# Zilong-Li/BaseVarC

Measured on AMD Instinct MI355X. Metric: sites/sec at N=1e6 samples; achieved HBM GB/s vs roofline, higher is better.
Workload: dtype f64

## Files before the change

### basevarc_amd/csrc/bvc_internal.h

```cpp
#pragma once
#include <hip/hip_runtime.h>
#include <stdint.h>

#include <vector>

#include "../../include/bvc.h"

namespace bvc {

struct LaunchState {
    int n_cu = 256;
    int em_waves_per_cu = 0;
    int em_wpb = 4;
    int hist_split = 0;
    int host_chunk_kib = 1 << 19;
    int em_streams = 0;
    int group_pipe = 1;
    int group_log2c = -1;
    int group_big_lds = 1;
    int group_h16 = 0;
    int em_engine = 0;
    int em_tiny_regions = 0;
    int csr_scatter_max = 64;
    int em_prune = 1;
    int stats_log2c = 2;
    int dbg_levels = 0;
    mutable uint32_t em_epoch = 0;
    struct RaisedLds { const void *kernel; size_t bytes; };
    mutable std::vector<RaisedLds> lds_raised;
};

inline size_t round256(size_t n) { return (n + 255) / 256 * 256; }

struct Layout {
    uintptr_t base = 0;
    size_t at = 0;
    template <class T> T *take(size_t count, size_t pad = 0)
    {
        T *p = reinterpret_cast<T *>(base + at);
        at += round256(count * sizeof(T) + pad);
        return p;
    }
};

hipError_t raise_lds(const LaunchState &st, const void *kernel, size_t bytes);

struct QualLut {
    double a[128];
    double e[128];
    double e_empty;
    double log_e[128];
    double log_a[128];
};

hipError_t launch_hist_dense(LaunchState &st, hipStream_t stream, int64_t n_sites, int64_t n_samples, int64_t row_stride,
                             const int8_t *bases, const int8_t *quals, const uint8_t *group_of_sample,
                             int n_groups, uint32_t *counts, int split, int64_t *group_scratch = nullptr,
                             uint8_t *hist_of_sample = nullptr);
constexpr int kGroupScratchWords = BVC_MAX_GROUPS + 4;
inline size_t group_redo_offset(int64_t n_samples) { return ((size_t)n_samples + 255) & ~(size_t)255; }
inline size_t group_labels_bytes(int64_t n_samples, int64_t n_sites) { return group_redo_offset(n_samples) + (size_t)n_sites + 256; }
int choose_hist_split(const LaunchState &st, int64_t n_sites, int64_t n_samples);

hipError_t launch_hist_packed(LaunchState &st, hipStream_t stream, int64_t n_sites, int64_t n_samples, int64_t row_stride,
                              const uint8_t *packed, uint32_t *counts, int split);
hipError_t launch_hist_packed_groups(LaunchState &st, hipStream_t stream, int64_t n_sites, int64_t n_samples,
                                     int64_t row_stride, const uint8_t *packed, const uint8_t *group_of_sample, int n_groups,
                                     uint32_t *counts, int64_t *group_scratch, uint8_t *hist_of_sample);
hipError_t launch_pack_dense(hipStream_t stream, int64_t n_sites, int64_t n_samples, int64_t stride_in, const int8_t *bases,
                             const int8_t *quals, int64_t stride_out, uint8_t *packed, unsigned long long *bad);

hipError_t launch_stream_read(hipStream_t stream, const void *src, int64_t bytes, uint32_t *sink);

hipError_t launch_hist_csr(LaunchState &st, hipStream_t stream, int64_t n_sites, const int64_t *offsets,
                           const int8_t *bases, const int8_t *quals, uint32_t *counts);

inline bool uses_item_engine(const LaunchState &st, double min_af) { return st.em_engine != 1 && min_af > 0.0; }
hipError_t launch_lrt(const LaunchState &st, hipStream_t stream, int64_t n_sites, const uint32_t *counts,
                      int64_t hist_stride, const int8_t *ref_base, double min_af, const QualLut *lut,
                      const int8_t *comb, const uint8_t *n_comb, bvc_site_result *results, bool shared = false,
                      int shared_waves_per_cu = 0,
                      void *scratch = nullptr);

size_t em_items_scratch_bytes(int64_t n_sites);
hipError_t launch_lrt_items(const LaunchState &st, hipStream_t stream, int64_t n_sites, int n_groups,
                            const uint32_t *counts, int64_t hist_stride, const int8_t *ref_base, double min_af,
                            const QualLut *lut, const int8_t *comb, const uint8_t *n_comb, bvc_site_result *results,
                            void *scratch, const uint8_t **taken_out, bool shared = false);

hipError_t launch_lrt_groups(const LaunchState &st, hipStream_t stream, int64_t n_sites, int n_groups,
                             const uint32_t *grp_counts, const int8_t *ref_base, double min_af, const QualLut *lut,
                             const bvc_site_result *overall, bvc_group_result *grp_results, bool shared = false,
                             int shared_waves_per_cu = 0, void *scratch = nullptr);
size_t em_group_scratch_bytes(int64_t n_sites, int n_groups);
constexpr int kGroupSharedWavesPerCu = 8;

hipError_t launch_sum_groups(hipStream_t stream, int64_t n_sites, int n_hist, const uint32_t *grp_counts,
                             uint32_t *counts);

hipError_t launch_synth_dense(hipStream_t stream, uint64_t seed, int64_t site0, int64_t n_sites,
                              int64_t n_samples, int64_t row_stride, uint32_t cov_thr16,
                              int8_t *bases, int8_t *quals, int8_t *ref_base);

struct PileupTile {
    const uint8_t *text = nullptr;
    bool bin = false;
    const uint32_t *line_start = nullptr;
    const int32_t *sample0 = nullptr, *n_in_batch = nullptr;
    int32_t n_batches = 0, n_pos = 0;
    int32_t line_stride = 0;
    const int32_t *n_pos_dev = nullptr;
    int64_t n_lines_cap = 0;
    uint32_t *line_words = nullptr;
    uint32_t *status = nullptr;
    int64_t *entry_off = nullptr, *obs_off = nullptr, *totals = nullptr;
    bvc_pileup_entry *entries = nullptr;
    int32_t *samples = nullptr;
    int8_t *obs_base = nullptr, *obs_qual = nullptr;
    const uint8_t *group_of_sample = nullptr;
    int64_t n_samples = 0;
    int32_t n_groups = 0;
    uint8_t *obs_label = nullptr;
    int32_t *tally = nullptr;
    bvc_pileup_indel *indels = nullptr;
    uint32_t indel_cap = 0;
};
struct bvc_pileup_region { uint32_t start, len, left_src, left_len; };
hipError_t launch_region_carry(hipStream_t stream, const uint8_t *old_text, uint8_t *text, const bvc_pileup_region *regions, int32_t n_batches);
hipError_t launch_region_index(hipStream_t stream, const PileupTile &P, const bvc_pileup_region *regions, const uint32_t *seg_base,
                               int64_t n_segments, uint32_t *seg_nl, int32_t *lines, int32_t max_pos);
hipError_t launch_region_ends(hipStream_t stream, const PileupTile &P, uint32_t *ends);
hipError_t launch_indel_text(hipStream_t stream, const PileupTile &P, uint8_t *dst, uint32_t dst_cap, uint32_t *used);
hipError_t launch_called_scan(hipStream_t stream, const PileupTile &P, const bvc_site_result *results, int64_t *called_off);
hipError_t launch_called_gather(hipStream_t stream, const PileupTile &P, const int64_t *called_off, bvc_pileup_entry *out_entries,
                                int32_t *out_samples);
hipError_t launch_pileup_count(hipStream_t stream, const PileupTile &P);
hipError_t launch_pileup_write(hipStream_t stream, const PileupTile &P, uint32_t carry_in);
hipError_t launch_hist_csr_groups(LaunchState &st, hipStream_t stream, int64_t n_sites, const int64_t *offsets, const int8_t *bases,
                                  const int8_t *quals, const int32_t *sample_of_obs, const uint8_t *group_of_sample, int64_t n_samples,
                                  int n_groups, uint32_t *counts);
hipError_t launch_hist_csr_labels(LaunchState &st, hipStream_t stream, int64_t n_sites, const int64_t *offsets, const uint8_t *obs,
                                  const uint8_t *quals, const uint8_t *group_of_obs, int n_groups, uint32_t *counts);

hipError_t launch_counts_add(hipStream_t stream, int64_t n_words, uint32_t *dst, const uint32_t *src);
hipError_t launch_hist_csr_scatter(const LaunchState &st, hipStream_t stream, int64_t n_sites, const int64_t *offsets, const uint8_t *obs,
                                   const uint8_t *quals, const uint8_t *group_of_obs, int n_groups, int64_t max_len, uint32_t *counts);
hipError_t launch_hist_csr_add(LaunchState &st, hipStream_t stream, int64_t n_sites, const int64_t *offsets, const uint8_t *obs,
                               const uint8_t *quals, const uint8_t *group_of_obs, int n_groups, int64_t min_len, uint32_t *counts);

constexpr int kStatsMaxLog2c = 4;
constexpr int kSiteStatsTrip = 4096;
hipError_t launch_site_stats(LaunchState &st, hipStream_t stream, int64_t n_sites, const int64_t *offsets, const bvc_pileup_entry *entries,
                             const int8_t *ref_base, const bvc_site_result *results, bvc_site_stats *stats);

hipError_t launch_inflate(hipStream_t stream, const uint8_t *comp, const bvc_bgzf_block *blocks, int64_t n_blocks, uint8_t *out, uint32_t *status);

#ifdef BVC_CHECK_LDS
hipError_t debug_read_inflate(uint32_t *out8, bool reset);
hipError_t debug_read_pileup(uint32_t *out8, bool reset);
hipError_t debug_read_site_stats(uint32_t *out8, bool reset);
hipError_t debug_read_hist(uint32_t *out8, bool reset);
hipError_t debug_read_wave_engine(uint32_t *out8, bool reset);
hipError_t debug_read_items(uint32_t *out8, bool reset);
#endif

}
```

### basevarc_amd/csrc/em_items.hip

```cpp
#include <algorithm>

#include "bvc_device.h"
#include "bvc_internal.h"
#include "em_common.h"

namespace bvc {
namespace {



constexpr int kTiny = 8, kNarrow = 32, kWide = 48;
template <int CPB> constexpr int site_table_bytes() { return 4 * CPB * 5; }

constexpr int kEmptyQ = 128;

struct FitItem {
    int32_t site;
    uint8_t base[4];
    double f0[4];
    double e_excl;
    double inv_n;
    double ll_excl;
};
static_assert(sizeof(FitItem) == 64, "FitItem layout");
// ... 420 lines not shown
        const FitItem *fi = items + item;
        const int base = fi->base[unit];
        if (base != 0xFF && BVC_LDS_OK(13, fi->site, kRegionSites) && BVC_LDS_OK(14, base, 4)) {
            active = true;
            fb = fi->f0[unit];
            const uint8_t *tab = cls + fi->site * site_table_bytes<CPB>();
            const uint32_t *tab_n = reinterpret_cast<const uint32_t *>(tab) + base * CPB + sub;
            const uint8_t *tab_q = tab + 16 * CPB + base * CPB + sub;
#pragma unroll
            for (int k = 0; k < kSlots; ++k) {
                n[k] = (double)tab_n[k * G];
                e[k] = lut_e[tab_q[k * G]];
            }
        }
    }
    if (!active) {
#pragma unroll
        for (int k = 0; k < kSlots; ++k) { n[k] = 0.0; e[k] = 0.25; }
    }

    double fprev = fb, dprev = 0.0;
    int it = 0;
    bool done = !valid;
    while (true) {
        double ta = fabs(fb - fprev) * dprev;
        const double e_excl = fi_c->e_excl, fb_scale = fi_c->inv_n;
        const double g = fma(-4.0, fb, 1.0);
        double ysum0 = 0.0, ysum1 = 0.0, acc_e0 = 0.0, acc_e1 = 0.0;
#ifdef BVC_RCP_CHUNK
        constexpr int CH = kSlots > BVC_RCP_CHUNK ? BVC_RCP_CHUNK : kSlots;
#else
        constexpr int CH = kSlots;
#endif
#pragma unroll
        for (int c0 = 0; c0 < kSlots; c0 += CH) {
            constexpr int kLast = kSlots % CH == 0 ? CH : kSlots % CH;
            if (c0 + CH <= kSlots) {
                double m[CH], y[CH];
#pragma unroll
                for (int k = 0; k < CH; ++k) m[k] = fma(g, e[c0 + k], fb);
                rcp_all<CH>(m, y);
#pragma unroll
                for (int k = 0; k < CH; k += 2) {
                    const double r0 = n[c0 + k] * y[k], r1 = n[c0 + k + 1] * y[k + 1];
                    ysum0 += r0; ysum1 += r1;
                    acc_e0 = fma(r0, e[c0 + k], acc_e0); acc_e1 = fma(r1, e[c0 + k + 1], acc_e1);
                }
            } else {
                double m[kLast], y[kLast];
#pragma unroll
                for (int k = 0; k < kLast; ++k) m[k] = fma(g, e[c0 + k], fb);
                rcp_all<kLast>(m, y);
#pragma unroll
                for (int k = 0; k < kLast; k += 2) {
                    const double r0 = n[c0 + k] * y[k], r1 = n[c0 + k + 1] * y[k + 1];
                    ysum0 += r0; ysum1 += r1;
                    acc_e0 = fma(r0, e[c0 + k], acc_e0); acc_e1 = fma(r1, e[c0 + k + 1], acc_e1);
                }
            }
        }
        const double acc_e = acc_e0 + acc_e1;
        const double acc_d = fma(-4.0, acc_e, ysum0 + ysum1);
        double etot = acc_e;
        item_sum2<ROWS, LOG2G>(etot, ta);
        const double dunit = unit_sum<LOG2G>(acc_d);
        const double ex = (fb * fb_scale) * (dunit + (etot + e_excl));
        const uint32_t a_hi = (uint32_t)__double2hiint(ta);
        bool conv = it > 0 && a_hi < kSureBelowHi;
        const bool straddle = !done && it > 0 && a_hi >= kSureBelowHi && a_hi < kSureAboveHi;
        if (__ballot(straddle) != 0) {
            double dl = 0.0;
            const double df = fb - fprev, gp = fma(-4.0, fprev, 1.0);
#pragma unroll
            for (int k = 0; k < kSlots; ++k) {
                const double mo = fma(gp, e[k], fprev);
                const double u = df * fma(-4.0, e[k], 1.0) * rcp_cubic(mo);
                double p = fma(-0.25, u, 1.0 / 3.0);
                p = fma(p, u, -0.5);
                p = fma(p, u, 1.0);
                dl = fma(n[k], fabs(u * p), dl);
            }
            dl = item_sum<ROWS, LOG2G>(dl);
            conv = conv || (straddle && dl < kEmEpsilon);
        }
        const bool stop = !done && (conv || it == kEmIters);
        if (__ballot(stop) != 0) {
            if (stop && sub == 0) {
                FitOut *o = outs + item;
                o->ex[unit] = active ? ex : 0.0;
                o->fl[unit] = fb;
                if (ROWS == 2) o->ex[unit + 2] = 0.0;
                if (unit == 0) { o->passes = it + 1; o->pad = 0; }
            }
            done = done || stop;
            if (__ballot(!done) == 0) break;
        }
        fprev = fb;
        dprev = acc_d;
        fb = ex;
        ++it;
    }
    {
        const double fl = outs[valid ? item : item0].fl[unit];
        const double g = fma(-4.0, fl, 1.0);
        double ll = 0.0;
#pragma unroll
        for (int k = 0; k < kSlots; ++k) {
            ll = fma(n[k], log_pos(fma(g, e[k], fl)), ll);
            if ((k & 3) == 3) __builtin_amdgcn_sched_barrier(0);
        }
        ll = item_sum<ROWS, LOG2G>(ll);
        if (valid && unit == 0 && sub == 0) outs[item].ll = ll + items[item].ll_excl;
    }
}

constexpr int kLog2G4 = 1, kLog2G2 = 2;
template <int CPB> constexpr int log2g4() { return CPB == kTiny ? 0 : kLog2G4; }
template <int CPB> constexpr int log2g2() { return CPB == kTiny ? 1 : kLog2G2; }
constexpr double kPruneSlackAbs = 1.0, kPruneSlackRel = 1e-6;

template <class RegionT>
__device__ __forceinline__ void site_decide(RegionT &R, int ls, int lane, int64_t site, int n_groups, int prune,
                                            const int8_t *__restrict__ ref_base, bvc_site_result *__restrict__ results)
{
    ItemSite S = R.site[ls];
    if (S.state != 1) {
        int zero = 0;
        asm volatile("" : "+v"(zero));
        if (lane == 0) { R.want[ls][0] = zero; R.want[ls][1] = zero; R.site[ls].n_emit = 0; }
        return;
    }
    uint32_t sets = 0;
    int n_emit = 0, p_deepest = 0;
    bool finished = false;

    auto fit_loglik = [&](int idx, double (&ex)[4], int &passes) -> double {
        if (!BVC_LDS_OK(15, idx, kPlaces)) idx = 0;
        const FitOut &o = R.outs[idx];
#pragma unroll
        for (int u = 0; u < 4; ++u) ex[u] = o.ex[u];
        passes = o.passes;
        return o.ll;
    };
    auto by_base = [&](uint32_t pm, const double (&ex)[4], double (&bp)[4]) {
#pragma unroll
        for (int j = 0; j < 4; ++j) bp[j] = 0.0;
        int u = 0;
#pragma unroll
        for (int p = 0; p < 4; ++p)
            if ((pm >> p) & 1u) {
                const int b = (S.blist >> (4 * p)) & 3u;
                const double v = u == 0 ? ex[0] : (u == 1 ? ex[1] : (u == 2 ? ex[2] : ex[3]));
                bp[0] = b == 0 ? v : bp[0]; bp[1] = b == 1 ? v : bp[1];
                bp[2] = b == 2 ? v : bp[2]; bp[3] = b == 3 ? v : bp[3];
                ++u;
            }
    };

    int first_sub = 0;
    if (S.first) {
        double ex[4];
        int passes = 0;
        S.lr_alt = fit_loglik(S.item[0], ex, passes);
        by_base((1u << S.n) - 1u, ex, S.base_frq);
        S.passes += passes; S.fits += 1;
        first_sub = 1;
        S.k = (int8_t)(S.n - 1);
        S.first = 0;
    }
    const int n = S.n, k = S.k;
    bool again = false;
    if (k < 1) {
        finished = true;
    } else if (k >= 2) {
        const int c_last = n - 1 - S.p_deepest;
        int i_min = S.best_i;
        double best_chi = S.best_chi, best_lr = S.best_lr;
        double best_bp[4] = {S.best_bp[0], S.best_bp[1], S.best_bp[2], S.best_bp[3]};
        if (!S.round2) {
            const uint32_t masks = S.sets >> (4 * first_sub);
            const int cnt = S.n_emit - first_sub;
#pragma unroll
            for (int c = 0; c < 3; ++c) {
                if (c >= cnt) break;
                const uint32_t pm = (masks >> (4 * c)) & 0xFu;
                double ex[4];
                int passes = 0;
                const double ll = fit_loglik(first_sub ? S.item[c + 1] : S.item[c], ex, passes);
                S.passes += passes; S.fits += 1;
                const double chi_c = 2.0 * (S.lr_alt - ll);
                if (c == 0 || chi_c < best_chi) {
                    best_chi = chi_c; best_lr = ll; i_min = (S.later && c >= c_last) ? c + 1 : c;
                    by_base(pm, ex, best_bp);
                }
            }
            if (S.later) {
                double u_c = 0.0;
                uint32_t in_set = 0;
#pragma unroll
                for (int p = 0; p < 4; ++p)
                    if ((S.later >> p) & 1u) in_set |= 1u << ((S.blist >> (4 * p)) & 3u);
#pragma unroll
                for (int b = 0; b < 4; ++b) u_c += ((in_set >> b) & 1u) ? 0.0 : S.lle[b];
                const double bound = 2.0 * (S.lr_alt - u_c);
                const bool ruled_out = prune && bound > best_chi + (kPruneSlackAbs + kPruneSlackRel * fabs(u_c)) && bound < __builtin_huge_val();
                again = !ruled_out;
            }
        } else {
            double ex[4];
            int passes = 0;
            const double ll = fit_loglik(S.item[0], ex, passes);
            S.passes += passes; S.fits += 1;
            const double chi_c = 2.0 * (S.lr_alt - ll);
            if (chi_c < best_chi || (chi_c == best_chi && c_last < i_min)) {
                best_chi = chi_c; best_lr = ll; i_min = c_last;
                by_base(S.later, ex, best_bp);
            }
        }
        if (again) {
            S.best_chi = best_chi; S.best_lr = best_lr; S.best_i = (int8_t)i_min;
#pragma unroll
            for (int j = 0; j < 4; ++j) S.best_bp[j] = best_bp[j];
            S.round2 = 1;
            sets = S.later; n_emit = 1; p_deepest = S.p_deepest;
        } else {
            S.round2 = 0;
            S.lr_alt = best_lr;
            S.chi = best_chi;
            if (best_chi < kLrtThreshold) {
                int cnt_all = 0;
                const uint32_t pm = (subset_masks(n, k, cnt_all) >> (4 * i_min)) & 0xFu;
                uint32_t nl = 0;
                int nn = 0;
#pragma unroll
                for (int p = 0; p < 4; ++p)
                    if ((pm >> p) & 1u) { nl |= ((S.blist >> (4 * p)) & 3u) << (4 * nn); ++nn; }
                S.blist = nl;
                S.n = (int8_t)k;
#pragma unroll
                for (int j = 0; j < 4; ++j) S.base_frq[j] = best_bp[j];
                S.k = (int8_t)(k - 1);
                S.later = 0;
                if (k - 1 >= 2) {
                    uint32_t later = 0;
                    p_deepest = deepest_position(S.depth, nl, k);
                    sets = level_subsets(k, p_deepest, n_emit, later);
                    S.later = (uint8_t)later;
                }
            } else {
                finished = true;
            }
        }
    }
    if (!finished && !again && S.k == 1) {
        const int b0 = (int)(S.blist & 3u), b1 = (int)((S.blist >> 4) & 3u);
        const double ll0 = single_allele_loglik(S.lla, S.lle, b0), ll1 = single_allele_loglik(S.lla, S.lle, b1);
        const double chi0 = 2.0 * (S.lr_alt - ll0), chi1 = 2.0 * (S.lr_alt - ll1);
        const bool second = chi1 < chi0;
        const double best_chi = second ? chi1 : chi0;
        const int bb = second ? b1 : b0;
        S.passes += 4; S.fits += 2;
        S.lr_alt = second ? ll1 : ll0;
        S.chi = best_chi;
        if (best_chi < kLrtThreshold) {
            S.blist = (uint32_t)bb;
            S.n = 1;
            S.base_frq[0] = bb == 0 ? 1.0 : 0.0; S.base_frq[1] = bb == 1 ? 1.0 : 0.0;
            S.base_frq[2] = bb == 2 ? 1.0 : 0.0; S.base_frq[3] = bb == 3 ? 1.0 : 0.0;
        }
        S.k = 0;
        finished = true;
    }
    S.sets = sets; S.n_emit = (int8_t)n_emit; S.p_deepest = (int8_t)p_deepest;
    int want[kLists];
    count_wanted(sets, n_emit, want);
    if (lane == 0) {
        if (finished) {
            store_record(results + site, S, (int)ref_base[ref_index(site, n_groups)], S.n, S.blist);
            S.state = 2;
        }
        R.site[ls] = S;
        R.want[ls][0] = want[0]; R.want[ls][1] = want[1];
    }
}

struct RegionArgs {
    int64_t n_sites;
    int n_groups;
    const uint32_t *counts;
    int64_t hist_stride;
    const QualLut *lut;
    const int8_t *ref_base;
    double min_af;
    const int8_t *comb;
    const uint8_t *n_comb;
    uint8_t *taken;
    bvc_site_result *results;
    uint32_t *kind_epoch;
    uint32_t epoch;
    int dbg_levels;
    int tiny_regions;
    int prune;
    int64_t region0;
};

__device__ __forceinline__ void wave_sync()
{
    __builtin_amdgcn_fence(__ATOMIC_RELEASE, "workgroup");
    __builtin_amdgcn_wave_barrier();
    __builtin_amdgcn_fence(__ATOMIC_ACQUIRE, "workgroup");
}

__device__ __forceinline__ void load_counts(uint32_t (&c)[8], const uint32_t *__restrict__ counts, int64_t hist_stride, int64_t site,
                                            int n_groups, int lane)
{
    const uint32_t *hist = counts + hist_index(site, n_groups) * hist_stride + (lane >> 4) * 128 + (lane & 15);
#pragma unroll
    for (int lvl = 0; lvl < 8; ++lvl) c[lvl] = hist[16 * lvl];
}

template <int TEAM, class RegionT>
__device__ __forceinline__ void team_sync(RegionT &R, uint32_t &phase, int lane)
{
    if (TEAM == 1) { wave_sync(); return; }
    __builtin_amdgcn_fence(__ATOMIC_RELEASE, "workgroup");
    __builtin_amdgcn_wave_barrier();
    phase += TEAM;
    if (lane == 0) {
        __hip_atomic_fetch_add(&R.arrive, 1u, __ATOMIC_RELEASE, __HIP_MEMORY_SCOPE_WORKGROUP);
        while (__hip_atomic_load(&R.arrive, __ATOMIC_ACQUIRE, __HIP_MEMORY_SCOPE_WORKGROUP) - phase > 0x7FFFFFFFu) __builtin_amdgcn_s_sleep(1);
    }
    __builtin_amdgcn_wave_barrier();
    __builtin_amdgcn_fence(__ATOMIC_ACQUIRE, "workgroup");
}

template <int CPB, int TEAM>
__device__ __forceinline__ void region_body(Region<CPB> *regions, const RegionArgs &A)
{
    const int wave = __builtin_amdgcn_readfirstlane((int)(threadIdx.x >> 6));
    const int teams = (int)(blockDim.x >> 6) / TEAM;
    const int member = wave % TEAM;
    const int lane = threadIdx.x & (kWave - 1);
    Region<CPB> &R = regions[wave / TEAM];
    const int64_t n_sites = A.n_sites;
    const int64_t n_regions = (n_sites + kRegionSites - 1) / kRegionSites;
    if (CPB == kWide && A.kind_epoch[1] != A.epoch) return;
    if (CPB == kTiny && A.kind_epoch[0] != A.epoch) return;
    uint32_t phase = 0;
    if (TEAM > 1) {
        if (member == 0 && lane == 0) R.arrive = 0u;
        __syncthreads();
    }
    const int64_t region = A.region0 + (int64_t)blockIdx.x * teams + wave / TEAM;
    for (bool first = true; region < n_regions && first; first = false) {
        const int64_t site0 = region * kRegionSites;
        if (member == 0 && lane == 0) { R.need = 0; R.next_slot = 0; }
        if (TEAM > 1) team_sync<TEAM>(R, phase, lane);
        int need = 0;
        uint32_t cnext[8];
        if (site0 + member < n_sites) load_counts(cnext, A.counts, A.hist_stride, site0 + member, A.n_groups, lane);
#pragma unroll 1
        for (int ls = member; ls < kRegionSites; ls += TEAM) {
            uint32_t c8[8];
#pragma unroll
            for (int k = 0; k < 8; ++k) c8[k] = cnext[k];
            if (ls + TEAM < kRegionSites && site0 + ls + TEAM < n_sites) load_counts(cnext, A.counts, A.hist_stride, site0 + ls + TEAM, A.n_groups, lane);
            if (site0 + ls < n_sites) {
                need = max(need, site_classes<CPB>(R, ls, lane, site0 + ls, c8, A.lut, A.min_af, A.comb, A.n_comb, A.taken));
            } else if (lane == 0) {
                R.site[ls].state = 2; R.site[ls].n_emit = 0;
                R.want[ls][0] = 0; R.want[ls][1] = 0;
            }
        }
        if (TEAM > 1) {
            if (lane == 0) atomicMax(&R.need, need);
            team_sync<TEAM>(R, phase, lane);
            need = R.need;
        } else {
            wave_sync();
        }
        const int kind = (A.tiny_regions && need <= kTiny) ? kTiny : (need <= kNarrow ? kNarrow : kWide);
        if (CPB == kNarrow && kind != kNarrow && member == 0 && lane == 0) A.kind_epoch[kind == kWide ? 1 : 0] = A.epoch;
        if (kind != CPB) {
            if (TEAM > 1) team_sync<TEAM>(R, phase, lane);
            continue;
        }
        if (member == 0 && lane < kRegionSites && R.site[lane].state == 3) {
            const int64_t site = site0 + lane;
            store_record(A.results + site, R.site[lane], (int)A.ref_base[ref_index(site, A.n_groups)], R.site[lane].n,
                         R.site[lane].blist);
            R.site[lane].state = 2;
        }
        team_sync<TEAM>(R, phase, lane);
        for (int round = 0; round < kRounds && round < (A.dbg_levels >> 1); ++round) {
            int cnt[kLists] = {0, 0};
#pragma unroll
            for (int w = 0; w < kRegionSites; ++w) {
#pragma unroll
                for (int l = 0; l < kLists; ++l) cnt[l] += R.want[w][l];
            }
            if (cnt[0] + cnt[1] == 0) break;
            const int first[kLists] = {0, cnt[0]};
            if (!BVC_LDS_OK(16, cnt[0] + cnt[1], kPlaces + 1)) break;
            if (member == 0) region_emit(R, lane, first);
            team_sync<TEAM>(R, phase, lane);
            constexpr int kPerWave4 = 16 >> log2g4<CPB>(), kPerWave2 = 2 * (16 >> log2g2<CPB>());
            const FitItem *items = R.items;
            FitOut *outs = R.outs;
            const uint8_t *tabs = &R.tab[0][0];
            const double *lut_e = A.lut->e;
            const int w0 = (cnt[0] + kPerWave4 - 1) / kPerWave4, w1 = w0 + (cnt[1] + kPerWave2 - 1) / kPerWave2;
            int slot = 0;
#pragma unroll 1
            for (;;) {
                if (TEAM > 1) {
                    if (lane == 0) slot = atomicAdd(&R.next_slot, 1);
                    slot = __builtin_amdgcn_readfirstlane(slot);
                }
                if (slot >= w1) break;
                if (slot < w0) fit_body<4, log2g4<CPB>(), CPB>(slot * kPerWave4, cnt[0], items, outs, tabs, lut_e);
                else fit_body<2, log2g2<CPB>(), CPB>(cnt[0] + (slot - w0) * kPerWave2, cnt[0] + cnt[1], items, outs, tabs, lut_e);
                if (TEAM == 1) ++slot;
            }
            team_sync<TEAM>(R, phase, lane);
            if (TEAM > 1 && member == 0 && lane == 0) R.next_slot = 0;
            if (round + 1 == (A.dbg_levels >> 1) && (A.dbg_levels & 1)) break;
            int my = lane;
            asm volatile("" : "+v"(my));
            if (member == 0 && my < kRegionSites && site0 + my < n_sites)
                site_decide(R, my, 0, site0 + my, A.n_groups, A.prune, A.ref_base, A.results);
            team_sync<TEAM>(R, phase, lane);
        }
        team_sync<TEAM>(R, phase, lane);
    }
}

#define BVC_OCCUPANCY(n) BVC_WAVES_PER_EU(n, n)
#ifdef BVC_RCP_CHUNK
#define BVC_REGION_WAVES_PER_EU 4
#else
#define BVC_REGION_WAVES_PER_EU 3
#endif
constexpr int kMaxRegionWaves = 4;
#ifndef BVC_REGION_TEAM
#define BVC_REGION_TEAM 2
#endif
constexpr int kTeam = BVC_REGION_TEAM;

template <int CPB>
__global__ __launch_bounds__(64 * kMaxRegionWaves) BVC_OCCUPANCY(CPB == kWide ? 2 : BVC_REGION_WAVES_PER_EU) void region_kernel(RegionArgs A)
{
    BVC_POISON_LDS();
    extern __shared__ __attribute__((aligned(16))) unsigned char region_lds[];
    region_body<CPB, kTeam>(reinterpret_cast<Region<CPB> *>(region_lds), A);
}

}

#ifdef BVC_CHECK_LDS
BVC_DEFINE_DEBUG_READER(debug_read_items)
#endif

struct ItemScratch {
    uint8_t *taken;
    uint32_t *kind_epoch;
};

static ItemScratch item_scratch(Layout &L, int64_t n_sites)
{
    const size_t start = L.at;
    ItemScratch s;
    s.taken = L.take<uint8_t>((size_t)n_sites);
    s.kind_epoch = L.take<uint32_t>(0);
    L.at = start + (size_t)n_sites + 256 + 64;
    return s;
}

size_t em_items_scratch_bytes(int64_t n_sites)
{
    Layout size;
    item_scratch(size, n_sites);
    return size.at;
}

hipError_t launch_lrt_items(const LaunchState &st, hipStream_t stream, int64_t n_sites, int n_groups,
                            const uint32_t *counts, int64_t hist_stride, const int8_t *ref_base, double min_af,
                            const QualLut *lut, const int8_t *comb, const uint8_t *n_comb, bvc_site_result *results,
                            void *scratch, const uint8_t **taken_out, bool shared)
{
    Layout slices{reinterpret_cast<uintptr_t>(scratch)};
    const ItemScratch scr = item_scratch(slices, n_sites);
    uint8_t *taken = scr.taken;
    const int64_t regions = (n_sites + kRegionSites - 1) / kRegionSites;
    int per_cu = 0;
    if (st.em_waves_per_cu > 0) per_cu = st.em_waves_per_cu;
    else if (shared) per_cu = 4;
    constexpr int kMaxTeams = kMaxRegionWaves / kTeam;
    int teams;
    int64_t wgs, per_launch;
    if (per_cu > 0) {
        const int want_teams = std::max(1, per_cu / kTeam);
        teams = std::min(want_teams, kMaxTeams);
        wgs = (regions + teams - 1) / teams;
        per_launch = (int64_t)st.n_cu * ((want_teams + teams - 1) / teams);
    } else {
        teams = (int)std::min<int64_t>(kMaxTeams, std::max<int64_t>(1, (regions + st.n_cu - 1) / st.n_cu));
        wgs = (regions + teams - 1) / teams;
        per_launch = wgs;
    }
    RegionArgs A;
    A.n_sites = n_sites; A.n_groups = n_groups; A.counts = counts; A.hist_stride = hist_stride; A.lut = lut;
    A.ref_base = ref_base; A.min_af = min_af; A.comb = comb; A.n_comb = n_comb; A.taken = taken; A.results = results;
    A.kind_epoch = scr.kind_epoch;
    A.epoch = ++st.em_epoch;
    if (A.epoch == 0) A.epoch = ++st.em_epoch;
    A.dbg_levels = st.dbg_levels > 0 ? st.dbg_levels : 2 * kRounds;
    A.tiny_regions = st.em_tiny_regions;
    A.prune = st.em_prune;
    A.region0 = 0;
    const hipError_t e = raise_lds(st, reinterpret_cast<const void *>(region_kernel<kWide>), kMaxTeams * sizeof(Region<kWide>));
    if (e != hipSuccess) return e;
    const dim3 block(64 * teams * kTeam);
    auto sequence = [&](auto kernel, size_t lds_per_team) {
        for (int64_t w0 = 0; w0 < wgs; w0 += per_launch) {
            A.region0 = w0 * teams;
            hipLaunchKernelGGL(kernel, dim3((unsigned)std::min(per_launch, wgs - w0)), block, teams * lds_per_team, stream, A);
        }
        A.region0 = 0;
    };
    sequence(region_kernel<kNarrow>, sizeof(Region<kNarrow>));
    if (st.em_tiny_regions) sequence(region_kernel<kTiny>, sizeof(Region<kTiny>));
    sequence(region_kernel<kWide>, sizeof(Region<kWide>));
    *taken_out = taken;
    return hipGetLastError();
}

}
```

### basevarc_amd/csrc/em_kernel.hip

```cpp
#include "bvc_device.h"
#include "bvc_internal.h"
#include "em_common.h"

namespace bvc {
namespace {

template <int NS>
struct Slots {
    double n[NS];
    double e[NS];
    double d[NS];
    double yp[NS];
};

struct Freq {
    double fb;
};

constexpr int kDppRor8 = 0x128;
constexpr int kDppRowBcast15 = 0x142;
template <int L> constexpr int dpp_newbcast() { return 0x150 + L; }

struct PassOut {
    double ex_own;
// ... 122 lines not shown

    int cnt_row = 0, depth_lane = 0;
#pragma unroll
    for (int lvl = 0; lvl < 8; ++lvl) {
        const int q = t + 16 * lvl;
        const uint32_t c = hist[row * 128 + q];
        const uint64_t nzmask = __ballot(c != 0);
        const uint32_t rowbits = (uint32_t)(nzmask >> (16 * row)) & 0xFFFFu;
        if (c != 0) {
            const int pos = cnt_row + __popc(rowbits & ((1u << t) - 1u));
            if (BVC_LDS_OK(21, pos, 128)) {
                s_n[row * 128 + pos] = c;
                s_q[row * 128 + pos] = (uint8_t)q;
            }
        }
        cnt_row += __popc(rowbits);
        depth_lane += (int)c;
    }
    const int depth_row = row_sum(depth_lane);
    int depth[4];
    depth[0] = __builtin_amdgcn_readlane(depth_row, 0);
    depth[1] = __builtin_amdgcn_readlane(depth_row, 16);
    depth[2] = __builtin_amdgcn_readlane(depth_row, 32);
    depth[3] = __builtin_amdgcn_readlane(depth_row, 48);
    int maxcnt = max(max(__builtin_amdgcn_readlane(cnt_row, 0), __builtin_amdgcn_readlane(cnt_row, 16)),
                     max(__builtin_amdgcn_readlane(cnt_row, 32), __builtin_amdgcn_readlane(cnt_row, 48)));
    const int nslots = (maxcnt + 15) >> 4;
    if (nslots > NS || (!ANY && NS > 2 && nslots <= NS / 2)) return false;
    wave_lds_sync<WPB>();

    Slots<NS> S;
#pragma unroll
    for (int k = 0; k < NS; ++k) {
        const int idx = t + 16 * k;
        S.n[k] = 0.0; S.d[k] = 0.0; S.e[k] = 1.0; S.yp[k] = 1.0;
        if (idx < cnt_row) {
            const int q = s_q[row * 128 + idx];
            S.n[k] = (double)s_n[row * 128 + idx];
            S.e[k] = lut->e[q];
            S.d[k] = lut->a[q] - S.e[k];
        }
    }

    const int total_i = depth[0] + depth[1] + depth[2] + depth[3];
    const double depth_total = (double)total_i;
    out = SiteOut{};
#pragma unroll
    for (int j = 0; j < 4; ++j) out.depth[j] = depth[j];
    out.depth_total = depth_total;
    if (total_i == 0) return true;
    const double inv_n = 1.0 / depth_total;

    uint32_t blist = 0;
    int n = 0;
    for (int c = 0; c < n_comb; ++c) {
        const int b = (comb_list >> (4 * c)) & 3;
        if ((double)pick4(depth, b) / depth_total >= min_af) { blist |= (uint32_t)b << (4 * n); ++n; }
    }
    if (n == 0) return true;

    int passes = 0, fits = 0;
    double base_frq[4] = {0, 0, 0, 0};
    double lr_alt = 0.0, chi = 0.0;
    int status = 0;

    auto fit_set = [&](uint32_t setmask, double &loglik, double (&ex)[4]) __attribute__((always_inline)) -> bool {
        int depth_sum = 0;
#pragma unroll
        for (int j = 0; j < 4; ++j) depth_sum += ((setmask >> j) & 1u) ? depth[j] : 0;
        double f[4];
#pragma unroll
        for (int j = 0; j < 4; ++j)
            f[j] = (depth_sum > 0 && ((setmask >> j) & 1u)) ? (double)depth[j] / (double)depth_sum : 0.0;
        const double freq_sum = ((f[0] + f[1]) + f[2]) + f[3];
        if (freq_sum == 0) return false;
        constexpr int kNarrow = NS == 2 ? 1 : (NS == 4 ? 3 : 6);
        if (kNarrow < NS && nslots <= kNarrow) loglik = em_fit<NS, kNarrow>(S, lane, pick4(f, row), inv_n, ex, passes);
        else loglik = em_fit<NS>(S, lane, pick4(f, row), inv_n, ex, passes);
        fits += 1;
        return true;
    };

    bool full_level = true;
    for (int k = n; k > 0; --k) {
        int ncomb = 0;
        const uint32_t masks = subset_masks(n, k, ncomb);
        int n_fit = 0, i_min = 0;
        double best_chi = 0.0, best_lr = 0.0, best_bp[4] = {0, 0, 0, 0};
        for (int c = 0; c < ncomb; ++c) {
            const uint32_t pm = (masks >> (4 * c)) & 0xFu;
            uint32_t setmask = 0;
            for (int p = 0; p < 4; ++p)
                if ((pm >> p) & 1u) setmask |= 1u << ((blist >> (4 * p)) & 3u);
            double ex[4], ll;
            if (!fit_set(setmask, ll, ex)) continue;
            const double chi_c = 2.0 * (lr_alt - ll);
            if (n_fit == 0 || chi_c < best_chi) {
                best_chi = chi_c; best_lr = ll; i_min = n_fit;
#pragma unroll
                for (int j = 0; j < 4; ++j) best_bp[j] = ex[j];
            }
            ++n_fit;
        }
        if (n_fit == 0) { status = 1; break; }
        lr_alt = best_lr;
        if (full_level) {
            full_level = false;
#pragma unroll
            for (int j = 0; j < 4; ++j) base_frq[j] = best_bp[j];
            continue;
        }
        chi = best_chi;
        if (chi < kLrtThreshold) {
            const uint32_t pm = (masks >> (4 * i_min)) & 0xFu;
            uint32_t nl = 0;
            int nn = 0;
            for (int p = 0; p < 4; ++p)
                if ((pm >> p) & 1u) { nl |= ((blist >> (4 * p)) & 3u) << (4 * nn); ++nn; }
            blist = nl;
            n = k;
#pragma unroll
            for (int j = 0; j < 4; ++j) base_frq[j] = best_bp[j];
        } else {
            break;
        }
    }
    if (status == 1 && full_level) { out.status = 1; out.n_passes = passes; out.n_fits = fits; return true; }

    out.status = status;
    out.n_passes = passes;
    out.n_fits = fits;
    out.lr_alt = lr_alt;
    out.chi = chi;
    out.n_kept = n;
#pragma unroll
    for (int j = 0; j < 4; ++j) { out.base_frq[j] = base_frq[j]; out.kept[j] = (j < n) ? (int)((blist >> (4 * j)) & 3u) : 0; }
    int n_alt = 0;
    int a0 = 0, a1 = 0, a2 = 0;
    double g0 = 0.0, g1 = 0.0, g2 = 0.0;
#pragma unroll
    for (int p = 0; p < 4; ++p) {
        const int b = (blist >> (4 * p)) & 3;
        if (p < n && b != ref && n_alt < 3) {
            const double fr = pick4(base_frq, b);
            if (n_alt == 0) { a0 = b; g0 = fr; } else if (n_alt == 1) { a1 = b; g1 = fr; } else { a2 = b; g2 = fr; }
            ++n_alt;
        }
    }
    out.alt_base[0] = a0; out.alt_base[1] = a1; out.alt_base[2] = a2;
    out.af[0] = g0; out.af[1] = g1; out.af[2] = g2;
    out.n_alt = n_alt;
    if (n_alt > 0) {
        out.var_qual = call_var_qual(n, pick4(depth, (int)(blist & 3u)), depth_total, chi);
        out.called = 1;
    }
    return true;
}

__device__ __forceinline__ void store_result(bvc_site_result *dst, const SiteOut &o)
{
    bvc_site_result r;
    r.var_qual = o.var_qual; r.chi = o.chi; r.depth_total = o.depth_total; r.lr_alt = o.lr_alt;
    for (int j = 0; j < 3; ++j) { r.af[j] = o.af[j]; r.alt_base[j] = (int8_t)o.alt_base[j]; }
    for (int j = 0; j < 4; ++j) { r.base_frq[j] = o.base_frq[j]; r.depth[j] = o.depth[j]; r.kept[j] = (int8_t)o.kept[j]; }
    r.n_passes = o.n_passes; r.n_alt = (uint8_t)o.n_alt; r.called = (uint8_t)o.called;
    r.n_kept = (uint8_t)o.n_kept; r.status = (uint8_t)o.status; r.n_fits = (uint8_t)o.n_fits;
    *dst = r;
}

template <int WPB>
__device__ __forceinline__ int wave_scratch(uint32_t (*&s_n_all)[512], uint8_t (*&s_q_all)[512])
{
    __shared__ uint32_t s_n[WPB][512];
    __shared__ uint8_t s_q[WPB][512];
    s_n_all = s_n;
    s_q_all = s_q;
    return WPB == 1 ? 0 : __builtin_amdgcn_readfirstlane((int)(threadIdx.x >> 6));
}

template <int NS, int WPB, bool ANY = false>
__global__ __launch_bounds__(64 * WPB) void lrt_kernel(int64_t n_sites, const uint32_t *__restrict__ counts,
                                                 int64_t hist_stride, const int8_t *__restrict__ ref_base,
                                                 double min_af, const QualLut *__restrict__ lut,
                                                 const int8_t *__restrict__ comb,
                                                 const uint8_t *__restrict__ n_comb,
                                                 const uint8_t *__restrict__ taken,
                                                 bvc_site_result *__restrict__ results)
{
    BVC_POISON_LDS();
    uint32_t (*s_n_all)[512];
    uint8_t (*s_q_all)[512];
    const int wave = wave_scratch<WPB>(s_n_all, s_q_all);
    for (int64_t site = (int64_t)blockIdx.x * WPB + wave; site < n_sites; site += (int64_t)gridDim.x * WPB) {
        if (taken && taken[site]) continue;
        uint32_t *s_n = s_n_all[wave];
        uint8_t *s_q = s_q_all[wave];
        uint32_t list = 0x3210u;
        int nc = 4;
        if (comb) {
            const int want = min((int)n_comb[site], 4);
            list = 0; nc = 0;
            for (int c = 0; c < want; ++c) {
                const int b = comb[site * 4 + c];
                if ((unsigned)b < 4u) { list |= (uint32_t)b << (4 * nc); ++nc; }
            }
        }
        SiteOut o;
        const bool mine = lrt_site<NS, WPB, ANY>(counts + site * hist_stride, ref_base[site], min_af, list, nc, lut, s_n, s_q, o);
        if (mine && (threadIdx.x & 63) == 0) store_result(results + site, o);
        wave_lds_sync<WPB>();
    }
}

template <int NS, int WPB, bool ANY = false>
__global__ __launch_bounds__(64 * WPB) void lrt_groups_kernel(int64_t n_sites, int n_groups,
                                                        const uint32_t *__restrict__ grp_counts,
                                                        const int8_t *__restrict__ ref_base, double min_af,
                                                        const QualLut *__restrict__ lut,
                                                        const bvc_site_result *__restrict__ overall,
                                                        const uint8_t *__restrict__ taken,
                                                        bvc_group_result *__restrict__ grp_results)
{
    BVC_POISON_LDS();
    uint32_t (*s_n_all)[512];
    uint8_t (*s_q_all)[512];
    const int wave = wave_scratch<WPB>(s_n_all, s_q_all);
    uint32_t *s_n = s_n_all[wave];
    uint8_t *s_q = s_q_all[wave];
    const int64_t n_work = n_sites * n_groups;
    for (int64_t w = (int64_t)blockIdx.x * WPB + wave; w < n_work; w += (int64_t)gridDim.x * WPB) {
        if (taken && taken[w]) continue;
        const int64_t site = w / n_groups;
        const int g = (int)(w % n_groups);
        const uint32_t *hist = grp_counts + (site * (n_groups + 1) + g) * BVC_NCLASS;
        if (!overall[site].called) {
            if (NS == 2 || ANY) {
                const int lane = threadIdx.x & 63, row = lane >> 4, t = lane & 15;
                int d = 0;
#pragma unroll
                for (int lvl = 0; lvl < 8; ++lvl) d += (int)hist[row * 128 + t + 16 * lvl];
                d = row_sum(d);
                const int d0 = __builtin_amdgcn_readlane(d, 0), d1 = __builtin_amdgcn_readlane(d, 16);
                const int d2 = __builtin_amdgcn_readlane(d, 32), d3 = __builtin_amdgcn_readlane(d, 48);
                if (lane == 0) grp_results[site * n_groups + g] = group_record_depths(d0, d1, d2, d3);
            }
            continue;
        }
        const bvc_site_result ov = overall[site];
        const int ref = ref_base[site];
        uint32_t list = (unsigned)ref < 4u ? (uint32_t)ref : 0u;
        int nc = (unsigned)ref < 4u ? 1 : 0;
#pragma unroll
        for (int i = 0; i < 3; ++i)
            if (i < ov.n_alt) { list |= (uint32_t)(ov.alt_base[i] & 3) << (4 * nc); ++nc; }
        SiteOut o;
        const bool mine = lrt_site<NS, WPB, ANY>(hist, ref, min_af, list, nc, lut, s_n, s_q, o);
        if (mine && (threadIdx.x & 63) == 0) {
            bvc_group_result r;
            for (int j = 0; j < 4; ++j) r.depth[j] = o.depth[j];
            for (int j = 0; j < 6; ++j) r.pad[j] = 0;
            r.ran = o.depth_total > 0 ? 1 : 0;
            r.present = 0;
#pragma unroll
            for (int i = 0; i < 3; ++i) {
                double af = 0.0;
                if (r.ran && i < ov.n_alt) {
#pragma unroll
                    for (int tt = 0; tt < 3; ++tt)
                        if (tt < o.n_alt && o.alt_base[tt] == ov.alt_base[i]) { af = o.af[tt]; r.present |= (uint8_t)(1u << i); }
                }
                r.af[i] = af;
            }
            grp_results[site * n_groups + g] = r;
        }
        wave_lds_sync<WPB>();
    }
}

__global__ void var_qual_kernel(int64_t n_sites, bvc_site_result *__restrict__ results)
{
    BVC_POISON_LDS();
    const int64_t s = (int64_t)blockIdx.x * blockDim.x + threadIdx.x;
    if (s >= n_sites) return;
    if (!results[s].called || results[s].var_qual != kVarQualPending) return;
    const double p = kf_gammaq_dev(0.5, results[s].chi / 2.0);
    double vq = (p != 0.0) ? -10 * log10(p) : 10000.0;
    if (vq == 0) vq = 0.0;
    results[s].var_qual = vq;
}

__global__ void sum_groups_kernel(int64_t total, int n_hist, const uint32_t *__restrict__ grp_counts,
                                  uint32_t *__restrict__ counts)
{
    BVC_POISON_LDS();
    const int64_t i = (int64_t)blockIdx.x * blockDim.x + threadIdx.x;
    if (i >= total) return;
    const int64_t site = i / BVC_NCLASS;
    const int key = (int)(i % BVC_NCLASS);
    uint32_t s = 0;
    for (int h = 0; h < n_hist; ++h) s += grp_counts[(site * n_hist + h) * BVC_NCLASS + key];
    counts[i] = s;
}

__global__ void group_comb_kernel(int64_t n_pseudo, int n_groups, const int8_t *__restrict__ ref_base,
                                  const bvc_site_result *__restrict__ overall, int8_t *__restrict__ comb,
                                  uint8_t *__restrict__ n_comb)
{
    BVC_POISON_LDS();
    const int64_t p = (int64_t)blockIdx.x * blockDim.x + threadIdx.x;
    if (p >= n_pseudo) return;
    const int64_t site = p / n_groups;
    int nc = 0;
    int8_t list[4] = {0, 0, 0, 0};
    if (overall[site].called) {
        const int ref = ref_base[site];
        if ((unsigned)ref < 4u) list[nc++] = (int8_t)ref;
        const int n_alt = overall[site].n_alt;
        for (int i = 0; i < 3; ++i)
            if (i < n_alt) list[nc++] = (int8_t)(overall[site].alt_base[i] & 3);
    }
    for (int c = 0; c < 4; ++c) comb[p * 4 + c] = list[c];
    n_comb[p] = (uint8_t)nc;
}

__global__ void group_records_kernel(int64_t n_pseudo, int n_groups, const bvc_site_result *__restrict__ overall,
                                     const bvc_site_result *__restrict__ pseudo, const uint8_t *__restrict__ taken,
                                     bvc_group_result *__restrict__ grp_results)
{
    BVC_POISON_LDS();
    const int64_t p = (int64_t)blockIdx.x * blockDim.x + threadIdx.x;
    if (p >= n_pseudo || !taken[p]) return;
    const int64_t site = p / n_groups;
    const bvc_site_result t = pseudo[p];
    bvc_group_result r;
    for (int j = 0; j < 4; ++j) r.depth[j] = t.depth[j];
    for (int j = 0; j < 6; ++j) r.pad[j] = 0;
    for (int j = 0; j < 3; ++j) r.af[j] = 0.0;
    r.ran = 0; r.present = 0;
    if (overall[site].called) {
        r.ran = t.depth_total > 0 ? 1 : 0;
        const int n_alt = overall[site].n_alt;
        for (int i = 0; i < 3; ++i)
            if (r.ran && i < n_alt)
                for (int tt = 0; tt < 3; ++tt)
                    if (tt < t.n_alt && t.alt_base[tt] == overall[site].alt_base[i]) { r.af[i] = t.af[tt]; r.present |= (uint8_t)(1u << i); }
    }
    grp_results[p] = r;
}

}

#ifdef BVC_CHECK_LDS
BVC_DEFINE_DEBUG_READER(debug_read_wave_engine)
#endif


static int64_t em_grid_cap(const LaunchState &st, bool shared, int shared_waves_per_cu = 0)
{
    int per_cu = shared ? (shared_waves_per_cu > 0 ? shared_waves_per_cu : 8) : 24;
    if (st.em_waves_per_cu > 0) per_cu = st.em_waves_per_cu;
    return (int64_t)per_cu * st.n_cu;
}

struct SiteKernels {
    template <int NS, int WPB, bool ANY = false> static constexpr auto kernel() { return lrt_kernel<NS, WPB, ANY>; }
};
struct GroupKernels {
    template <int NS, int WPB, bool ANY = false> static constexpr auto kernel() { return lrt_groups_kernel<NS, WPB, ANY>; }
};

template <class Family, int WPB, class... Args>
static void launch_variants(hipStream_t stream, int64_t want_waves, const uint8_t *taken, Args... args)
{
    const dim3 grid((unsigned)((want_waves + WPB - 1) / WPB)), block(64 * WPB);
    if (taken) {
        hipLaunchKernelGGL((Family::template kernel<8, WPB, true>()), grid, block, 0, stream, args...);
        return;
    }
    hipLaunchKernelGGL((Family::template kernel<2, WPB>()), grid, block, 0, stream, args...);
    hipLaunchKernelGGL((Family::template kernel<4, WPB>()), grid, block, 0, stream, args...);
    hipLaunchKernelGGL((Family::template kernel<8, WPB>()), grid, block, 0, stream, args...);
}

template <class Family, class... Args>
static void launch_wave_kernels(const LaunchState &st, hipStream_t stream, int64_t n_work, bool shared, int shared_waves_per_cu,
                                const uint8_t *taken, Args... args)
{
    const int64_t cap = em_grid_cap(st, shared, shared_waves_per_cu);
    const int64_t want_waves = n_work < cap ? n_work : cap;
    if (st.em_wpb == 1) launch_variants<Family, 1>(stream, want_waves, taken, args...);
    else launch_variants<Family, 4>(stream, want_waves, taken, args...);
}

template <class Kernel, class... Args>
static void launch_per_element(Kernel kernel, hipStream_t stream, int64_t n, Args... args)
{
    hipLaunchKernelGGL(kernel, dim3((unsigned)((n + 255) / 256)), dim3(256), 0, stream, n, args...);
}

hipError_t launch_lrt(const LaunchState &st, hipStream_t stream, int64_t n_sites, const uint32_t *counts,
                      int64_t hist_stride, const int8_t *ref_base, double min_af, const QualLut *lut,
                      const int8_t *comb, const uint8_t *n_comb, bvc_site_result *results, bool shared,
                      int shared_waves_per_cu, void *scratch)
{
    if (n_sites <= 0) return hipSuccess;
    const uint8_t *taken = nullptr;
    if (scratch && uses_item_engine(st, min_af)) {
        const hipError_t e = launch_lrt_items(st, stream, n_sites, 0, counts, hist_stride, ref_base, min_af, lut, comb, n_comb,
                                              results, scratch, &taken, shared);
        if (e != hipSuccess) return e;
    }
    launch_wave_kernels<SiteKernels>(st, stream, n_sites, shared, shared_waves_per_cu, taken, n_sites, counts, hist_stride, ref_base,
                                     min_af, lut, comb, n_comb, taken, results);
    launch_per_element(var_qual_kernel, stream, n_sites, results);
    return hipGetLastError();
}

struct GroupScratch {
    int8_t *comb;
    uint8_t *n_comb;
    bvc_site_result *pseudo;
    void *items;
};

static GroupScratch group_scratch(Layout &L, int64_t n_pseudo)
{
    GroupScratch s;
    s.comb = L.take<int8_t>((size_t)n_pseudo * 4);
    s.n_comb = L.take<uint8_t>((size_t)n_pseudo);
    s.pseudo = L.take<bvc_site_result>((size_t)n_pseudo);
    s.items = L.take<char>(0);
    L.at += em_items_scratch_bytes(n_pseudo);
    return s;
}

size_t em_group_scratch_bytes(int64_t n_sites, int n_groups)
{
    Layout size;
    group_scratch(size, n_sites * n_groups);
    return size.at;
}

hipError_t launch_lrt_groups(const LaunchState &st, hipStream_t stream, int64_t n_sites, int n_groups,
                             const uint32_t *grp_counts, const int8_t *ref_base, double min_af, const QualLut *lut,
                             const bvc_site_result *overall, bvc_group_result *grp_results, bool shared,
                             int shared_waves_per_cu, void *scratch)
{
    if (n_sites <= 0 || n_groups <= 0) return hipSuccess;
    const int64_t n_work = n_sites * n_groups;
    const uint8_t *taken = nullptr;
    if (scratch && uses_item_engine(st, min_af)) {
        Layout slices{reinterpret_cast<uintptr_t>(scratch)};
        const GroupScratch s = group_scratch(slices, n_work);
        launch_per_element(group_comb_kernel, stream, n_work, n_groups, ref_base, overall, s.comb, s.n_comb);
        const hipError_t e = launch_lrt_items(st, stream, n_work, n_groups, grp_counts, BVC_NCLASS, ref_base, min_af, lut, s.comb,
                                              s.n_comb, s.pseudo, s.items, &taken, shared);
        if (e != hipSuccess) return e;
        launch_per_element(group_records_kernel, stream, n_work, n_groups, overall, s.pseudo, taken, grp_results);
    }
    launch_wave_kernels<GroupKernels>(st, stream, n_work, shared, shared_waves_per_cu, taken, n_sites, n_groups, grp_counts, ref_base,
                                      min_af, lut, overall, taken, grp_results);
    return hipGetLastError();
}

hipError_t launch_sum_groups(hipStream_t stream, int64_t n_sites, int n_hist, const uint32_t *grp_counts,
                             uint32_t *counts)
{
    const int64_t total = n_sites * BVC_NCLASS;
    if (total <= 0) return hipSuccess;
    launch_per_element(sum_groups_kernel, stream, total, n_hist, grp_counts, counts);
    return hipGetLastError();
}

}
```

Before: 3.369 million.

## Compact group EM work to called sites via live index list

Replaces the per-pseudo-site comb kernel with a kernel that ranks called sites, writes a compacted list of live (site, group) indices, and clears the taken flags. The item EM region kernel and group records kernel then iterate only over that index list, so uncalled sites skip histogram loads and class work. This adds an O(blocks × sites) prefix count per block (each block rescans all preceding sites), an extra indirection in the EM inner loop, and device-side reads of the live count.

Result: no change. 3.366 million (-0.1%).

```diff
diff --git a/basevarc_amd/csrc/bvc_internal.h b/basevarc_amd/csrc/bvc_internal.h
--- a/basevarc_amd/csrc/bvc_internal.h
+++ b/basevarc_amd/csrc/bvc_internal.h
@@ -83,10 +83,12 @@
                       void *scratch = nullptr);
 
 size_t em_items_scratch_bytes(int64_t n_sites);
+uint8_t *em_items_taken(void *scratch, int64_t n_sites);
 hipError_t launch_lrt_items(const LaunchState &st, hipStream_t stream, int64_t n_sites, int n_groups,
                             const uint32_t *counts, int64_t hist_stride, const int8_t *ref_base, double min_af,
                             const QualLut *lut, const int8_t *comb, const uint8_t *n_comb, bvc_site_result *results,
-                            void *scratch, const uint8_t **taken_out, bool shared = false);
+                            void *scratch, const uint8_t **taken_out, bool shared = false, const uint32_t *index = nullptr,
+                            const uint32_t *n_index = nullptr);
 
 hipError_t launch_lrt_groups(const LaunchState &st, hipStream_t stream, int64_t n_sites, int n_groups,
                              const uint32_t *grp_counts, const int8_t *ref_base, double min_af, const QualLut *lut,
diff --git a/basevarc_amd/csrc/em_items.hip b/basevarc_amd/csrc/em_items.hip
--- a/basevarc_amd/csrc/em_items.hip
+++ b/basevarc_amd/csrc/em_items.hip
@@ -746,7 +746,14 @@
     int tiny_regions;
     int prune;
     int64_t region0;
+    const uint32_t *index;
+    const uint32_t *n_index;
 };
+
+__device__ __forceinline__ int64_t site_at(const RegionArgs &A, int64_t j)
+{
+    return A.index ? (int64_t)A.index[j] : j;
+}
 
 __device__ __forceinline__ void wave_sync()
 {
@@ -786,8 +793,9 @@
     const int member = wave % TEAM;
     const int lane = threadIdx.x & (kWave - 1);
     Region<CPB> &R = regions[wave / TEAM];
-    const int64_t n_sites = A.n_sites;
+    const int64_t n_sites = A.index ? (int64_t)*A.n_index : A.n_sites;
     const int64_t n_regions = (n_sites + kRegionSites - 1) / kRegionSites;
+    if (A.index && A.region0 + (int64_t)blockIdx.x * teams >= n_regions) return;
     if (CPB == kWide && A.kind_epoch[1] != A.epoch) return;
     if (CPB == kTiny && A.kind_epoch[0] != A.epoch) return;
     uint32_t phase = 0;
@@ -802,15 +810,16 @@
         if (TEAM > 1) team_sync<TEAM>(R, phase, lane);
         int need = 0;
         uint32_t cnext[8];
-        if (site0 + member < n_sites) load_counts(cnext, A.counts, A.hist_stride, site0 + member, A.n_groups, lane);
+        if (site0 + member < n_sites) load_counts(cnext, A.counts, A.hist_stride, site_at(A, site0 + member), A.n_groups, lane);
 #pragma unroll 1
         for (int ls = member; ls < kRegionSites; ls += TEAM) {
             uint32_t c8[8];
 #pragma unroll
             for (int k = 0; k < 8; ++k) c8[k] = cnext[k];
-            if (ls + TEAM < kRegionSites && site0 + ls + TEAM < n_sites) load_counts(cnext, A.counts, A.hist_stride, site0 + ls + TEAM, A.n_groups, lane);
+            if (ls + TEAM < kRegionSites && site0 + ls + TEAM < n_sites)
+                load_counts(cnext, A.counts, A.hist_stride, site_at(A, site0 + ls + TEAM), A.n_groups, lane);
             if (site0 + ls < n_sites) {
-                need = max(need, site_classes<CPB>(R, ls, lane, site0 + ls, c8, A.lut, A.min_af, A.comb, A.n_comb, A.taken));
+                need = max(need, site_classes<CPB>(R, ls, lane, site_at(A, site0 + ls), c8, A.lut, A.min_af, A.comb, A.n_comb, A.taken));
             } else if (lane == 0) {
                 R.site[ls].state = 2; R.site[ls].n_emit = 0;
                 R.want[ls][0] = 0; R.want[ls][1] = 0;
@@ -830,7 +839,7 @@
             continue;
         }
         if (member == 0 && lane < kRegionSites && R.site[lane].state == 3) {
-            const int64_t site = site0 + lane;
+            const int64_t site = site_at(A, site0 + lane);
             store_record(A.results + site, R.site[lane], (int)A.ref_base[ref_index(site, A.n_groups)], R.site[lane].n,
                          R.site[lane].blist);
             R.site[lane].state = 2;
@@ -872,7 +881,7 @@
             int my = lane;
             asm volatile("" : "+v"(my));
             if (member == 0 && my < kRegionSites && site0 + my < n_sites)
-                site_decide(R, my, 0, site0 + my, A.n_groups, A.prune, A.ref_base, A.results);
+                site_decide(R, my, 0, site_at(A, site0 + my), A.n_groups, A.prune, A.ref_base, A.results);
             team_sync<TEAM>(R, phase, lane);
         }
         team_sync<TEAM>(R, phase, lane);
@@ -927,10 +936,16 @@
     return size.at;
 }
 
+uint8_t *em_items_taken(void *scratch, int64_t n_sites)
+{
+    Layout slices{reinterpret_cast<uintptr_t>(scratch)};
+    return item_scratch(slices, n_sites).taken;
+}
+
 hipError_t launch_lrt_items(const LaunchState &st, hipStream_t stream, int64_t n_sites, int n_groups,
                             const uint32_t *counts, int64_t hist_stride, const int8_t *ref_base, double min_af,
                             const QualLut *lut, const int8_t *comb, const uint8_t *n_comb, bvc_site_result *results,
-                            void *scratch, const uint8_t **taken_out, bool shared)
+                            void *scratch, const uint8_t **taken_out, bool shared, const uint32_t *index, const uint32_t *n_index)
 {
     Layout slices{reinterpret_cast<uintptr_t>(scratch)};
     const ItemScratch scr = item_scratch(slices, n_sites);
@@ -962,6 +977,7 @@
     A.tiny_regions = st.em_tiny_regions;
     A.prune = st.em_prune;
     A.region0 = 0;
+    A.index = index; A.n_index = n_index;
     const hipError_t e = raise_lds(st, reinterpret_cast<const void *>(region_kernel<kWide>), kMaxTeams * sizeof(Region<kWide>));
     if (e != hipSuccess) return e;
     const dim3 block(64 * teams * kTeam);
diff --git a/basevarc_amd/csrc/em_kernel.hip b/basevarc_amd/csrc/em_kernel.hip
--- a/basevarc_amd/csrc/em_kernel.hip
+++ b/basevarc_amd/csrc/em_kernel.hip
@@ -448,34 +448,62 @@
     counts[i] = s;
 }
 
-__global__ void group_comb_kernel(int64_t n_pseudo, int n_groups, const int8_t *__restrict__ ref_base,
-                                  const bvc_site_result *__restrict__ overall, int8_t *__restrict__ comb,
-                                  uint8_t *__restrict__ n_comb)
+constexpr int kLiveBlock = 256;
+__global__ __launch_bounds__(kLiveBlock) void group_live_kernel(int64_t n_sites, int n_groups, const int8_t *__restrict__ ref_base,
+                                                                 const bvc_site_result *__restrict__ overall,
+                                                                 int8_t *__restrict__ comb, uint8_t *__restrict__ n_comb,
+                                                                 uint8_t *__restrict__ taken, uint32_t *__restrict__ live,
+                                                                 uint32_t *__restrict__ n_live)
 {
     BVC_POISON_LDS();
-    const int64_t p = (int64_t)blockIdx.x * blockDim.x + threadIdx.x;
-    if (p >= n_pseudo) return;
-    const int64_t site = p / n_groups;
+    __shared__ uint32_t s_wave[kLiveBlock / kWave];
+    __shared__ uint32_t s_before[kLiveBlock / kWave];
+    const int tid = (int)threadIdx.x, lane = tid & (kWave - 1), wave = tid >> 6;
+    const int64_t first = (int64_t)blockIdx.x * kLiveBlock;
+    const int64_t site = first + tid;
+    uint32_t before = 0;
+    for (int64_t s = tid; s < first; s += kLiveBlock) before += overall[s].called ? 1u : 0u;
+    const bool called = site < n_sites && overall[site].called;
+    const uint64_t votes = __ballot(called);
+    for (int off = 32; off > 0; off >>= 1) before += __shfl_xor(before, off, kWave);
+    if (lane == 0) { s_wave[wave] = (uint32_t)__popcll(votes); s_before[wave] = before; }
+    __syncthreads();
+    uint32_t rank = 0, total = 0;
+    for (int w = 0; w < kLiveBlock / kWave; ++w) {
+        rank += s_before[w] + (w < wave ? s_wave[w] : 0u);
+        total += s_before[w] + s_wave[w];
+    }
+    rank += (uint32_t)__popcll(votes & ((1ull << lane) - 1ull));
+    if (blockIdx.x == gridDim.x - 1 && tid == 0) *n_live = total * (uint32_t)n_groups;
+    if (site >= n_sites) return;
+    const int64_t p0 = site * n_groups;
+    for (int g = 0; g < n_groups; ++g) taken[p0 + g] = 0;
+    if (!called) return;
     int nc = 0;
     int8_t list[4] = {0, 0, 0, 0};
-    if (overall[site].called) {
-        const int ref = ref_base[site];
-        if ((unsigned)ref < 4u) list[nc++] = (int8_t)ref;
-        const int n_alt = overall[site].n_alt;
-        for (int i = 0; i < 3; ++i)
-            if (i < n_alt) list[nc++] = (int8_t)(overall[site].alt_base[i] & 3);
-    }
-    for (int c = 0; c < 4; ++c) comb[p * 4 + c] = list[c];
-    n_comb[p] = (uint8_t)nc;
+    const int ref = ref_base[site];
+    if ((unsigned)ref < 4u) list[nc++] = (int8_t)ref;
+    const int n_alt = overall[site].n_alt;
+    for (int i = 0; i < 3; ++i)
+        if (i < n_alt) list[nc++] = (int8_t)(overall[site].alt_base[i] & 3);
+    for (int g = 0; g < n_groups; ++g) {
+        const int64_t p = p0 + g;
+        for (int c = 0; c < 4; ++c) comb[p * 4 + c] = list[c];
+        n_comb[p] = (uint8_t)nc;
+        live[(int64_t)rank * n_groups + g] = (uint32_t)p;
+    }
 }
 
 __global__ void group_records_kernel(int64_t n_pseudo, int n_groups, const bvc_site_result *__restrict__ overall,
                                      const bvc_site_result *__restrict__ pseudo, const uint8_t *__restrict__ taken,
+                                     const uint32_t *__restrict__ live, const uint32_t *__restrict__ n_live,
                                      bvc_group_result *__restrict__ grp_results)
 {
     BVC_POISON_LDS();
-    const int64_t p = (int64_t)blockIdx.x * blockDim.x + threadIdx.x;
-    if (p >= n_pseudo || !taken[p]) return;
+    const int64_t i = (int64_t)blockIdx.x * blockDim.x + threadIdx.x;
+    if (i >= n_pseudo || i >= (int64_t)*n_live) return;
+    const int64_t p = live[i];
+    if (!taken[p]) return;
     const int64_t site = p / n_groups;
     const bvc_site_result t = pseudo[p];
     bvc_group_result r;
@@ -566,6 +594,8 @@
     int8_t *comb;
     uint8_t *n_comb;
     bvc_site_result *pseudo;
+    uint32_t *live;
+    uint32_t *n_live;
     void *items;
 };
 
@@ -575,6 +605,8 @@
     s.comb = L.take<int8_t>((size_t)n_pseudo * 4);
     s.n_comb = L.take<uint8_t>((size_t)n_pseudo);
     s.pseudo = L.take<bvc_site_result>((size_t)n_pseudo);
+    s.live = L.take<uint32_t>((size_t)n_pseudo);
+    s.n_live = L.take<uint32_t>(1);
     s.items = L.take<char>(0);
     L.at += em_items_scratch_bytes(n_pseudo);
     return s;
@@ -598,11 +630,12 @@
     if (scratch && uses_item_engine(st, min_af)) {
         Layout slices{reinterpret_cast<uintptr_t>(scratch)};
         const GroupScratch s = group_scratch(slices, n_work);
-        launch_per_element(group_comb_kernel, stream, n_work, n_groups, ref_base, overall, s.comb, s.n_comb);
+        hipLaunchKernelGGL(group_live_kernel, dim3((unsigned)((n_sites + kLiveBlock - 1) / kLiveBlock)), dim3(kLiveBlock), 0, stream,
+                           n_sites, n_groups, ref_base, overall, s.comb, s.n_comb, em_items_taken(s.items, n_work), s.live, s.n_live);
         const hipError_t e = launch_lrt_items(st, stream, n_work, n_groups, grp_counts, BVC_NCLASS, ref_base, min_af, lut, s.comb,
-                                              s.n_comb, s.pseudo, s.items, &taken, shared);
+                                              s.n_comb, s.pseudo, s.items, &taken, shared, s.live, s.n_live);
         if (e != hipSuccess) return e;
-        launch_per_element(group_records_kernel, stream, n_work, n_groups, overall, s.pseudo, taken, grp_results);
+        launch_per_element(group_records_kernel, stream, n_work, n_groups, overall, s.pseudo, taken, s.live, s.n_live, grp_results);
     }
     launch_wave_kernels<GroupKernels>(st, stream, n_work, shared, shared_waves_per_cu, taken, n_sites, n_groups, grp_counts, ref_base,
                                       min_af, lut, overall, taken, grp_results);
```
